# XinkeAE/Active-ORB-SLAM2

Hardware: AMD Instinct MI355X
Metric: frames/sec (extract+match+localBA) TUM 640x480 (higher is better)
Workload: dtype u8 (extract, match) + f64 (PoseOptimization, LocalBA)

## Files before the change

active-orb-slam2_amd/csrc/lba.hip:

```cpp
#include <dlfcn.h>

#include <chrono>
#include <cstdio>
#include <cstdlib>
#include <memory>
#include <numeric>
#include <atomic>
#include <condition_variable>
#include <functional>
#include <mutex>
#include <thread>

#include "lba_math.h"
#include "ldlt_reg.h"
#include "wave_ops.h"

namespace aos2 {

struct Cam {
    double fx, fy, cx, cy, bf;
    float bf_f;
    double delta_mono, delta_stereo;
};

struct LmState {
    double lambda, ni, currentChi, iniChi;
    double final_chi2, final_lambda;
    int32_t phase;
    int32_t run;
    int32_t lin;
    int32_t initp;
    int32_t xmark;
    int32_t it, qmax, nBad;
    int32_t iters_max[2], iters_done[2], trials[2];
    int32_t polls;
    int32_t stop_poll;
    int32_t stop_at_poll;
    int32_t n_active;
    int32_t solver_failed;
    int32_t blocks_done;
    int32_t ntr;
    int32_t err_at;
    int32_t pad_;
    double tr_rho[48], tr_temp[48], tr_cur[48], tr_lambda[48];
};

enum LdltForm : int { kLdltDev = 0, kLdltReg = 2 };

struct LbaWin {
    int n_poses, n_points, n_edges, np, nl, n_items;
    int iters1, iters2;
    const float *in_Tcw, *in_xyz, *in_obs, *in_w;
    double *pose, *point;
    double *bk;
    int est_n;
    const int32_t *e_pose, *e_point;
    const uint8_t *e_stereo;
    uint8_t *e_robust, *e_level1;
    double *err;
    Cam cam;
    const int32_t *pl_pos;
    const int32_t *hpose, *hpoint;
    const int32_t *pt_off, *pt_k;
    const int32_t *ps_off, *ps_k;
    const int32_t *pl_off, *pl_ph;
    const int32_t *it_ka, *it_kb, *it_l, *blk_off;
    const int32_t *sr_o0, *sr_info, *sr_ij;
    int n_srows;
    double *lrec;
    double *lomr;
    double *Rl;
    double *Hpp, *Hll, *b, *x, *Hs, *bs;
    double *tmp;
    double *scal;
    double *part;
    int n_part;
    double *ldlt;
    int npad;
    LdltForm ldlt_form;
    int hs_ld;
    LmState *st;
    const int32_t *abort_word;
    float *out_Tcw, *out_xyz;
    double *out_chi2;
    uint8_t *out_outlier;
};

static_assert(sizeof(LbaWin) == 520 && offsetof(LbaWin, st) == 472, "LbaWin's layout is fixed");

struct SchurTask {
    int32_t w;
    int32_t code;
};

__device__ inline bool lm_poll(LmState *st, const int32_t *abort_word, int seen = -1)
{
    st->polls++;
    if (st->stop_poll > 0) return true;
    const int a = seen >= 0 ? seen : abort_word ? __hip_atomic_load(abort_word, __ATOMIC_RELAXED, __HIP_MEMORY_SCOPE_SYSTEM) : 0;
    if (a || (st->stop_at_poll > 0 && st->polls >= st->stop_at_poll)) {
        st->stop_poll = st->polls;
        return true;
    }
    return false;
}

__device__ inline void lm_first_done(LmState *st, const int32_t *abort_word, int seen = -1)
{
    st->phase = 1;
    st->xmark = 0;
    if (lm_poll(st, abort_word, seen)) {
        st->phase = 3;
        return;
    }
    st->xmark = 1;
    st->n_active = 0;
}

template <int N>
__device__ __forceinline__ void workgroup_sum2(double v0, double v1, double *out0, double *out1)
{
    __shared__ double sh[2][N];
    sh[0][threadIdx.x] = v0;
    sh[1][threadIdx.x] = v1;
    __syncthreads();
#pragma unroll
    for (int s = N / 2; s > 0; s >>= 1) {
        if ((int)threadIdx.x < s) {
            sh[0][threadIdx.x] = sh[0][threadIdx.x] + sh[0][threadIdx.x + s];
            sh[1][threadIdx.x] = sh[1][threadIdx.x] + sh[1][threadIdx.x + s];
        }
        __syncthreads();
    }
    if (threadIdx.x == 0) {
        out0[blockIdx.x] = sh[0][0];
        out1[blockIdx.x] = sh[1][0];
    }
}

__global__ __launch_bounds__(256) void k_prepare(const LbaWin *__restrict__ wins, int stop_at_poll)
{
    const LbaWin &W = wins[blockIdx.y];
    const int i = blockIdx.x * 256 + threadIdx.x;
    if (i < W.n_poses) pose_from_Tcw(W.in_Tcw + 16 * (size_t)i, W.pose + 7 * (size_t)i);
    if (i < W.n_points)
        for (int d = 0; d < 3; ++d) W.point[3 * (size_t)i + d] = (double)W.in_xyz[3 * (size_t)i + d];
    if (i < W.n_edges) {
        for (int d = 0; d < 3; ++d) W.err[3 * (size_t)i + d] = 0.0;
        W.e_robust[i] = 1;
        W.e_level1[i] = 0;
    }
    if (blockIdx.x == 0 && W.hs_ld == W.npad) {
        const int n = 6 * W.np, npad = W.npad;
        for (int q = threadIdx.x; q < (npad - n) * npad; q += 256) {
            const int r = n + q / npad, c = q % npad;
            W.Hs[(size_t)r * npad + c] = r == c ? 1.0 : 0.0;
        }
        for (int q = threadIdx.x; q < n * (npad - n); q += 256) {
            const int r = q / (npad - n), c = n + q % (npad - n);
            W.Hs[(size_t)r * npad + c] = 0.0;
        }
    }
    if (blockIdx.x == 0) {
        LmState *st = W.st;
        static_assert(sizeof(LmState) % 8 == 0, "LmState is cleared as 64-bit words");
        for (int k = threadIdx.x; k < (int)(sizeof(LmState) / 8); k += 256) reinterpret_cast<long long *>(st)[k] = 0;
        __syncthreads();
        if (threadIdx.x == 0) {
            st->iters_max[0] = W.iters1;
            st->iters_max[1] = W.iters2;
            st->polls = 1;
            st->stop_at_poll = stop_at_poll;
            st->n_active = W.n_edges;
            st->phase = 0;
            st->it = 0;
            if (st->iters_max[0] <= 0 || lm_poll(st, W.abort_word)) {
                st->iters_done[0] = 0;
                lm_first_done(st, W.abort_word);
            } else
                st->initp = 1;
        }
    }
}
// ... 347 lines not shown
            const int a = e0 + kLmSlots * rd + j;
            double c = 0;
            if (a < e1) {
                const int e = W.pt_k[a];
                if (!W.e_level1[e]) {
                    double p[3], er[3];
                    se3_map(W.pose + 7 * (size_t)W.e_pose[e], Xv, p);
                    const int stereo = W.e_stereo[e];
                    const double ob[3] = {(double)W.in_obs[3 * (size_t)e], (double)W.in_obs[3 * (size_t)e + 1], (double)W.in_obs[3 * (size_t)e + 2]};
                    edge_error(W.cam, p, ob, stereo, er);
                    c = edge_chi2(er, (double)W.in_w[e], stereo ? 3 : 2);
                    if (W.e_robust[e]) {
                        double rho[2];
                        robustify(c, stereo ? W.cam.delta_stereo : W.cam.delta_mono, rho);
                        c = rho[0];
                    }
                }
            }
            s_v[ll][j][0] = c;
            __syncthreads();
            if (leader) {
                const int m = min(kLmSlots, e1 - (e0 + kLmSlots * rd));
                for (int jj = 0; jj < m; ++jj) chi += s_v[ll][jj][0];
            }
        }
    }
    if (has && leader) {
        store_dev(W.part + l, chi);
        store_dev(W.part + W.nl + l, sc);
    }
    if (solve) points_tail<256>(W);
}

__global__ __launch_bounds__(128) void k_points_walk(const LbaWin *__restrict__ wins, const SchurTask *__restrict__ tasks, int solve)
{
    const SchurTask tk = tasks[blockIdx.x];
    const LbaWin &W = wins[tk.w];
    if (!(solve ? W.st->run : W.st->initp)) return;
    const int l = tk.code * blockDim.x + threadIdx.x;
    const int n6 = 6 * W.np;
    if (l < W.nl) {
        double sc = 0, chi = 0;
        double *X = W.point + 3 * (size_t)W.hpoint[l];
        double Xv[3] = {X[0], X[1], X[2]};
        if (solve) {
            const double lambda = W.st->lambda;
            double cl[3] = {W.b[n6 + 3 * l], W.b[n6 + 3 * l + 1], W.b[n6 + 3 * l + 2]};
            const int a0 = W.pl_off[l], a1 = W.pl_off[l + 1];
            for (int a = a0; a < a1; a += kWalkChunk) {
                int ka[kWalkChunk], i1[kWalkChunk];
#pragma unroll
                for (int u = 0; u < kWalkChunk; ++u) ka[u] = min(a + u, a1 - 1);
#pragma unroll
                for (int u = 0; u < kWalkChunk; ++u) i1[u] = W.pl_ph[ka[u]];
                dbl4_t rec[kWalkChunk];
                double xp[kWalkChunk][6], Rr[kWalkChunk][9];
#pragma unroll
                for (int u = 0; u < kWalkChunk; ++u) rec[u] = lrec_load(W, ka[u]);
#pragma unroll
                for (int u = 0; u < kWalkChunk; ++u) {
#pragma unroll
                    for (int r = 0; r < 6; ++r) xp[u][r] = -W.x[6 * i1[u] + r];
#pragma unroll
                    for (int i = 0; i < 9; ++i) Rr[u][i] = W.Rl[9 * (size_t)i1[u] + i];
                }
#pragma unroll
                for (int u = 0; u < kWalkChunk; ++u) {
                    if (a + u >= a1) break;
                    double v[3];
                    lrec_backsub(W.cam, rec[u], Rr[u], xp[u], v);
                    for (int c = 0; c < 3; ++c) cl[c] += v[c];
                }
            }
            double Dm[9], Dinv[9];
            for (int i = 0; i < 9; ++i) Dm[i] = W.Hll[9 * (size_t)l + i];
            Dm[0] += lambda; Dm[4] += lambda; Dm[8] += lambda;
            mat3_inverse(Dm, Dinv);
            double *Xb = W.bk + 7 * (size_t)W.n_poses + 3 * (size_t)W.hpoint[l];
            for (int r = 0; r < 3; ++r) {
                const double xl = Dinv[r * 3] * cl[0] + Dinv[r * 3 + 1] * cl[1] + Dinv[r * 3 + 2] * cl[2];
                W.x[n6 + 3 * l + r] = xl;
                store_dev(Xb + r, Xv[r]);
                Xv[r] += xl;
                store_dev(X + r, Xv[r]);
                sc += xl * (lambda * xl + W.b[n6 + 3 * l + r]);
            }
        }
        const int e0 = W.pt_off[l], e1 = W.pt_off[l + 1];
        for (int a = e0; a < e1; a += kWalkChunkE) {
            int e[kWalkChunkE], ep[kWalkChunkE];
            uint8_t lv1[kWalkChunkE], ste[kWalkChunkE], rob[kWalkChunkE];
            double T[kWalkChunkE][7], ob[kWalkChunkE][3], ew[kWalkChunkE];
#pragma unroll
            for (int u = 0; u < kWalkChunkE; ++u) e[u] = W.pt_k[min(a + u, e1 - 1)];
#pragma unroll
            for (int u = 0; u < kWalkChunkE; ++u) {
                ep[u] = W.e_pose[e[u]];
                lv1[u] = W.e_level1[e[u]];
                ste[u] = W.e_stereo[e[u]];
                rob[u] = W.e_robust[e[u]];
                ew[u] = (double)W.in_w[e[u]];
#pragma unroll
                for (int i = 0; i < 3; ++i) ob[u][i] = (double)W.in_obs[3 * (size_t)e[u] + i];
            }
#pragma unroll
            for (int u = 0; u < kWalkChunkE; ++u)
#pragma unroll
                for (int i = 0; i < 7; ++i) T[u][i] = W.pose[7 * (size_t)ep[u] + i];
#pragma unroll
            for (int u = 0; u < kWalkChunkE; ++u) {
                if (a + u >= e1) break;
                if (lv1[u]) continue;
                double p[3], er[3];
                se3_map(T[u], Xv, p);
                const int stereo = ste[u];
                edge_error(W.cam, p, ob[u], stereo, er);
                double c = edge_chi2(er, ew[u], stereo ? 3 : 2);
                if (rob[u]) {
                    double rho[2];
                    robustify(c, stereo ? W.cam.delta_stereo : W.cam.delta_mono, rho);
                    c = rho[0];
                }
                chi += c;
            }
        }
        store_dev(W.part + l, chi);
        store_dev(W.part + W.nl + l, sc);
    }
    if (solve) points_tail<128>(W);
}

__device__ __forceinline__ void edge_weights_of(const Cam &cam, const double er[3], double w, int robust, int stereo, double omr[3], double &wo)
{
    omr[0] = -(w * er[0]);
    omr[1] = -(w * er[1]);
    omr[2] = stereo ? -(w * er[2]) : 0.0;
    wo = w;
    if (robust) {
        double rho[2];
        robustify(edge_chi2(er, w, stereo ? 3 : 2), stereo ? cam.delta_stereo : cam.delta_mono, rho);
        wo = rho[1] * w;
        omr[0] *= rho[1];
        omr[1] *= rho[1];
        if (stereo) omr[2] *= rho[1];
    }
}
__device__ __forceinline__ void edge_weights(const LbaWin &W, int k, const double p[3], int stereo, double omr[3], double &wo)
{
    const double ob[3] = {(double)W.in_obs[3 * (size_t)k], (double)W.in_obs[3 * (size_t)k + 1], (double)W.in_obs[3 * (size_t)k + 2]};
    double er[3];
    edge_error(W.cam, p, ob, stereo, er);
    edge_weights_of(W.cam, er, (double)W.in_w[k], W.e_robust[k], stereo, omr, wo);
}

__device__ __forceinline__ void lin_points_body(const LbaWin &W, int blk)
{
    __shared__ double s_c[kLmBlock][kLmSlots][12 + 1];
    const int tid = threadIdx.x, ll = tid / kLmSlots, j = tid % kLmSlots;
    const int l = blk * kLmBlock + ll;
    const bool has = l < W.nl, leader = j == 0;
    double Xv[3] = {0, 0, 0};
// ... 17 lines not shown
            jac_point(W.cam, R, p, stereo, Ja);
            double omr[3], wo;
            edge_weights(W, k, p, stereo, omr, wo);
#pragma unroll
            for (int r = 0; r < 3; ++r) {
                cb[r] = Ja[r] * omr[0] + Ja[3 + r] * omr[1] + Ja[6 + r] * omr[2];
#pragma unroll
                for (int c = 0; c < 3; ++c) cH[r * 3 + c] = Ja[r] * wo * Ja[c] + Ja[3 + r] * wo * Ja[3 + c] + Ja[6 + r] * wo * Ja[6 + c];
            }
            const int pp = W.pl_pos[k];
            if (pp >= 0) lrec_store(W, pp, p, wo, stereo, omr);
        }
#pragma unroll
        for (int i = 0; i < 9; ++i) s_c[ll][j][i] = cH[i];
#pragma unroll
        for (int i = 0; i < 3; ++i) s_c[ll][j][9 + i] = cb[i];
        __syncthreads();
        if (leader) {
            const int m = min(kLmSlots, a1 - (a0 + kLmSlots * rd));
            for (int jj = 0; jj < m; ++jj) {
#pragma unroll
                for (int i = 0; i < 9; ++i) H[i] += s_c[ll][jj][i];
#pragma unroll
                for (int i = 0; i < 3; ++i) bl[i] += s_c[ll][jj][9 + i];
            }
        }
    }
    if (has && leader) {
        for (int i = 0; i < 9; ++i) W.Hll[9 * (size_t)l + i] = H[i];
        for (int i = 0; i < 3; ++i) W.b[6 * (size_t)W.np + 3 * (size_t)l + i] = bl[i];
    }
}

__device__ __forceinline__ void lin_points_walk(const LbaWin &W, int l)
{
    if (l >= W.nl) return;
    const double *X = W.point + 3 * (size_t)W.hpoint[l];
    const double Xv[3] = {X[0], X[1], X[2]};
    double H[9] = {0, 0, 0, 0, 0, 0, 0, 0, 0}, bl[3] = {0, 0, 0};
    const int e0 = W.pt_off[l], e1 = W.pt_off[l + 1];
    for (int a = e0; a < e1; a += kWalkChunkLin) {
        int kk[kWalkChunkLin], ep[kWalkChunkLin], ph[kWalkChunkLin];
        uint8_t lv1[kWalkChunkLin], ste[kWalkChunkLin], rob[kWalkChunkLin];
        double T[kWalkChunkLin][7], er[kWalkChunkLin][3], ew[kWalkChunkLin];
#pragma unroll
        for (int u = 0; u < kWalkChunkLin; ++u) kk[u] = W.pt_k[min(a + u, e1 - 1)];
#pragma unroll
        for (int u = 0; u < kWalkChunkLin; ++u) {
            ep[u] = W.e_pose[kk[u]];
            ph[u] = W.pl_pos[kk[u]];
            lv1[u] = W.e_level1[kk[u]];
            ste[u] = W.e_stereo[kk[u]];
            rob[u] = W.e_robust[kk[u]];
            ew[u] = (double)W.in_w[kk[u]];
#pragma unroll
            for (int i = 0; i < 3; ++i) er[u][i] = (double)W.in_obs[3 * (size_t)kk[u] + i];
        }
#pragma unroll
        for (int u = 0; u < kWalkChunkLin; ++u)
#pragma unroll
            for (int i = 0; i < 7; ++i) T[u][i] = W.pose[7 * (size_t)ep[u] + i];
#pragma unroll
        for (int u = 0; u < kWalkChunkLin; ++u) {
            if (a + u >= e1) break;
            if (lv1[u]) continue;
            const int stereo = ste[u];
            double p[3], R[9];
            se3_map(T[u], Xv, p);
            rot_from_quat(T[u], R);
            double Ja[9];
            jac_point(W.cam, R, p, stereo, Ja);
            double omr[3], wo;
            double res[3];
            edge_error(W.cam, p, er[u], stereo, res);
            edge_weights_of(W.cam, res, ew[u], rob[u], stereo, omr, wo);
#pragma unroll
            for (int r = 0; r < 3; ++r) {
                bl[r] += Ja[r] * omr[0] + Ja[3 + r] * omr[1] + Ja[6 + r] * omr[2];
#pragma unroll
                for (int c = 0; c < 3; ++c) H[r * 3 + c] += Ja[r] * wo * Ja[c] + Ja[3 + r] * wo * Ja[3 + c] + Ja[6 + r] * wo * Ja[6 + c];
            }
            if (ph[u] >= 0) lrec_store(W, ph[u], p, wo, stereo, omr);
        }
    }
    for (int i = 0; i < 9; ++i) W.Hll[9 * (size_t)l + i] = H[i];
    for (int i = 0; i < 3; ++i) W.b[6 * (size_t)W.np + 3 * (size_t)l + i] = bl[i];
}

template <int K, int NT = 256>
__device__ __forceinline__ double workgroup_sum_k256(double (&acc)[K], double *red , int n_items)
{
    const int row = threadIdx.x >> 4, wave = threadIdx.x >> 6;
    const int rows_used = min(NT / 16, (n_items + 15) >> 4);
    if (wave * 64 < n_items) {
        row_sums_scatter_f64<K>(acc);
        row_scatter_store<K>(acc, red + row * (K + 1));
    }
    __syncthreads();
    double sum = 0;
    if ((int)threadIdx.x < K)
        for (int r = 0; r < rows_used; ++r) sum += red[r * (K + 1) + threadIdx.x];
    return sum;
}

__device__ __forceinline__ void lin_poses_body(const LbaWin &W, int ph, int init)
{
    __shared__ double red[16 * 43];
    if (ph >= W.np) return;
    double T[7];
    {
        const double *Tp = W.pose + 7 * (size_t)W.hpose[ph];
#pragma unroll
        for (int i = 0; i < 7; ++i) T[i] = Tp[i];
    }
    if (threadIdx.x == 0) {
        double R[9];
        rot_from_quat(T, R);
// ... 6 lines not shown
    for (int i = 0; i < 42; ++i) acc[i] = 0;
    for (int a = W.ps_off[ph] + threadIdx.x; a < W.ps_off[ph + 1]; a += 256) {
        const int k = W.ps_k[a];
        if (W.e_level1[k]) continue;
        const int stereo = W.e_stereo[k];
        double p[3], Jb[18], omr[3], wo;
        se3_map(T, W.point + 3 * (size_t)W.e_point[k], p);
        jac_pose(W.cam, p, stereo, Jb);
        edge_weights(W, k, p, stereo, omr, wo);
#pragma unroll
        for (int r = 0; r < 6; ++r) {
            acc[36 + r] += Jb[r] * omr[0] + Jb[6 + r] * omr[1] + Jb[12 + r] * omr[2];
#pragma unroll
            for (int c = 0; c < 6; ++c) acc[r * 6 + c] += Jb[r] * wo * Jb[c] + Jb[6 + r] * wo * Jb[6 + c] + Jb[12 + r] * wo * Jb[12 + c];
        }
    }
    const double sum = workgroup_sum_k256<42>(acc, red, W.ps_off[ph + 1] - W.ps_off[ph]);
    if (threadIdx.x < 36)
        W.Hpp[36 * (size_t)ph + threadIdx.x] = sum;
    else if (threadIdx.x < 42)
        W.b[6 * (size_t)ph + (threadIdx.x - 36)] = sum;
}

template <bool kWalk>
__global__ __launch_bounds__(256) __attribute__((amdgpu_waves_per_eu(3, 3))) void k_lin(const LbaWin *__restrict__ wins, const SchurTask *__restrict__ tasks, int init)
{
    const SchurTask tk = tasks[blockIdx.x];
    const LbaWin &W = wins[tk.w];
    if (!(init ? W.st->initp : W.st->lin)) return;
    const int blk = tk.code & 0x0fffffff;
    const bool keyframe = (tk.code >> 28) != 0;
    if (keyframe)
        lin_poses_body(W, blk, init);
    else if (kWalk)
        lin_points_walk(W, blk * 256 + threadIdx.x);
    else
        lin_points_body(W, blk);
}

__global__ __launch_bounds__(1024) void k_lm_init(const LbaWin *__restrict__ wins)
{
    __shared__ double sh[1024];
    const LbaWin &W = wins[blockIdx.x];
    LmState *st = W.st;
    if (!st->initp) return;
    const int n6 = 6 * W.np, n = n6 + 3 * W.nl;
    double acc = 0;
    for (int i = threadIdx.x; i < n; i += 1024) {
        double v;
        if (i < n6)
            v = W.Hpp[36 * (size_t)(i / 6) + (i % 6) * 7];
        else {
            const int j = i - n6;
            v = W.Hll[9 * (size_t)(j / 3) + (j % 3) * 4];
        }
        acc = fmax(acc, fabs(v));
    }
    sh[threadIdx.x] = acc;
    __syncthreads();
    for (int s = 512; s > 0; s >>= 1) {
        if ((int)threadIdx.x < s) sh[threadIdx.x] = fmax(sh[threadIdx.x], sh[threadIdx.x + s]);
        __syncthreads();
    }
    for (int i = threadIdx.x; i < W.est_n; i += 1024) W.bk[i] = W.pose[i];
    double chi, unused;
    canonical_sums(W, false, chi, unused);
    if (threadIdx.x == 0) {
        st->currentChi = st->iniChi = chi;
        st->lambda = 1e-5 * sh[0];
// ... 510 lines not shown
        for (int i = 0; i < 6; ++i) {
            upd[i] = xs[6 * tid + i];
            Wn.tmp[6 * tid + i] = upd[i] * (lambda * upd[i] + Wn.b[6 * tid + i]);
        }
        double *Tp = Wn.pose + 7 * (size_t)Wn.hpose[tid], *Tbk = Wn.bk + 7 * (size_t)Wn.hpose[tid];
        for (int i = 0; i < 7; ++i) Tbk[i] = Tp[i];
        se3_oplus_fast(upd, Tp);
    }
}

__device__ __forceinline__ void edge_last_error(const LbaWin &W, int e, int at, const double p_cur[3], int stereo, bool keep, double er[3])
{
    double *dst = W.err + 3 * (size_t)e;
    if (at == 0) {
        er[0] = dst[0]; er[1] = dst[1]; er[2] = dst[2];
        return;
    }
    double p[3] = {p_cur[0], p_cur[1], p_cur[2]};
    if (at == 2) se3_map(W.bk + 7 * (size_t)W.e_pose[e], W.bk + 7 * (size_t)W.n_poses + 3 * (size_t)W.e_point[e], p);
    const double ob[3] = {(double)W.in_obs[3 * (size_t)e], (double)W.in_obs[3 * (size_t)e + 1], (double)W.in_obs[3 * (size_t)e + 2]};
    edge_error(W.cam, p, ob, stereo, er);
    if (keep) {
        dst[0] = er[0]; dst[1] = er[1]; dst[2] = er[2];
    }
}

__global__ __launch_bounds__(256) void k_transition(const LbaWin *__restrict__ wins)
{
    __shared__ int s_last;
    const LbaWin &W = wins[blockIdx.y];
    LmState *st = W.st;
    if (!st->xmark) return;
    const int err_at = st->err_at;
    const int e = blockIdx.x * blockDim.x + threadIdx.x;
    int keep = 0;
    if (e < W.n_edges) {
        const int stereo = W.e_stereo[e];
        double p[3], er[3];
        se3_map(W.pose + 7 * (size_t)W.e_pose[e], W.point + 3 * (size_t)W.e_point[e], p);
        edge_last_error(W, e, err_at, p, stereo, true, er);
        const double c = edge_chi2(er, (double)W.in_w[e], stereo ? 3 : 2);
        const bool bad = c > (stereo ? 7.815 : 5.991) || !(p[2] > 0.0);
        if (bad) {
            W.e_level1[e] = 1;
            const int pp = W.pl_pos[e];
            if (pp >= 0) lrec_mask(W, pp);
        }
        W.e_robust[e] = 0;
        keep = bad ? 0 : 1;
    }
    const unsigned long long m = __ballot(keep);
    if ((threadIdx.x & 63) == 0 && m) atomicAdd(&st->n_active, __popcll(m));
    asm volatile("s_waitcnt vmcnt(0)" ::: "memory");
    __syncthreads();
    if (threadIdx.x == 0) s_last = __hip_atomic_fetch_add(&st->blocks_done, 1, __ATOMIC_RELAXED, __HIP_MEMORY_SCOPE_AGENT) == (int)gridDim.x - 1;
    __syncthreads();
    if (!s_last || threadIdx.x != 0) return;
    st->blocks_done = 0;
    st->xmark = 0;
    st->it = 0;
    st->err_at = 0;
    const int n_active = __hip_atomic_load(&st->n_active, __ATOMIC_RELAXED, __HIP_MEMORY_SCOPE_AGENT);
    if (n_active == 0 || st->iters_max[1] <= 0 || lm_poll(st, W.abort_word)) {
        st->phase = 3;
        st->iters_done[1] = 0;
    } else {
        st->phase = 2;
        st->initp = 1;
    }
}

__global__ __launch_bounds__(256) void k_final(const LbaWin *__restrict__ wins)
{
    const LbaWin &W = wins[blockIdx.y];
    const int i = blockIdx.x * blockDim.x + threadIdx.x;
    if (i < W.n_edges) {
        const int stereo = W.e_stereo[i];
        double p[3], er[3];
        se3_map(W.pose + 7 * (size_t)W.e_pose[i], W.point + 3 * (size_t)W.e_point[i], p);
        edge_last_error(W, i, W.e_level1[i] ? 0 : W.st->err_at, p, stereo, false, er);
        const double c = edge_chi2(er, (double)W.in_w[i], stereo ? 3 : 2);
// ... 254 lines not shown
    const int np = S.np;
    for (int i = 0; i < np; ++i) S.units.push_back((kSchurDiag << 28) | i);
    std::vector<int32_t> pack_first;
    int in_unit = 0;
    for (int i1 = 0, blk = 0; i1 < np; ++i1)
        for (int i2 = i1; i2 < np; ++i2, ++blk) {
            if (i2 == i1) continue;
            const int o0 = S.blk_off[blk], n = S.blk_off[blk + 1] - o0;
            if (n > 256) {
                S.units.push_back((kSchurBig << 28) | blk);
                continue;
            }
            const int nrows = std::max(1, (n + 15) / 16);
            if (in_unit + nrows > 16) {
                for (; in_unit < 16; ++in_unit) {
                    S.sr_o0.push_back(0); S.sr_info.push_back(0); S.sr_ij.push_back(0);
                }
                in_unit = 0;
            }
            if (in_unit == 0) pack_first.push_back((int32_t)S.sr_o0.size());
            for (int r = 0; r < nrows; ++r) {
                S.sr_o0.push_back(o0 + 16 * r);
                S.sr_info.push_back(std::max(0, std::min(16, n - 16 * r)) | (r << 8) | (nrows << 16));
                S.sr_ij.push_back(i1 | (i2 << 16));
            }
            in_unit = (in_unit + nrows) % 16;
        }
    for (int32_t f : pack_first) S.units.push_back((kSchurPack << 28) | f);
}

struct WinLayout {
    size_t in_Tcw, in_xyz, in_obs, in_w, e_pose, e_point, e_stereo, pl_pos, hpose, hpoint, pt_off, pt_k, ps_off, ps_k,
        pl_off, pl_k, it_ka, it_kb, it_l, blk_off, sr_o0, sr_info, sr_ij;
    size_t est, bk, robust, level1, err, lrec, lomr, Rl, Hpp, Hll, b, x, Hs, bs, tmp, scal, part, ldlt;
    size_t out_Tcw, out_xyz, out_outlier, out_chi2, st;
    int n_part, npad;
    LdltForm ldlt_form;
    size_t n_items;
};

struct RoctxRange {
    typedef int (*push_t)(const char *);
    typedef int (*pop_t)();
    static void resolve(push_t &push, pop_t &pop)
    {
        static push_t s_push = nullptr;
        static pop_t s_pop = nullptr;
        static bool tried = false;
        if (!tried) {
            tried = true;
            const char *v = getenv("AOS2_ROCTX");
            if (v && atoi(v) != 0) {
                void *h = dlopen("librocprofiler-sdk-roctx.so", RTLD_NOW | RTLD_GLOBAL);
                if (!h) h = dlopen("libroctx64.so", RTLD_NOW | RTLD_GLOBAL);
                if (h) {
                    s_push = (push_t)dlsym(h, "roctxRangePushA");
                    s_pop = (pop_t)dlsym(h, "roctxRangePop");
                }
            }
        }
        push = s_push;
        pop = s_pop;
    }
    pop_t pop_ = nullptr;
    explicit RoctxRange(const char *name)
    {
        push_t push;
// ... 76 lines not shown
    list(l.blk_off, S.blk_off, 4);
    list(l.sr_o0, S.sr_o0, 4); list(l.sr_info, S.sr_info, 4); list(l.sr_ij, S.sr_ij, 4);
}

static void layout_staged(const aos2_lba_problem_t &p, const Pass &S, Bump &B, WinLayout &l)
{
    for_each_staged(p, S, l, [&](size_t &off, const void *, size_t bytes, size_t tail) { off = B.take(bytes + tail); });
    l.n_items = S.it_ka.size();
}

static void stage_window(uint8_t *dst, const WinLayout &l, const aos2_lba_problem_t &p, const Pass &S)
{
    for_each_staged(p, S, l, [&](size_t off, const void *src, size_t bytes, size_t) {
        if (bytes) memcpy(dst + off, src, bytes);
    });
}

static void layout_scratch(const aos2_lba_problem_t &p, const Pass &S, const LmLayout &lay, Bump &B, WinLayout &l)
{
    const size_t NP = p.n_poses, NL = p.n_points, E = p.n_edges;
    const size_t n6 = 6 * (size_t)S.np, dim = n6 + 3 * (size_t)S.nl;
    l.est = B.take(8 * (7 * NP + 3 * NL)); l.bk = B.take(8 * (7 * NP + 3 * NL));
    l.robust = B.take(E); l.level1 = B.take(E);
    l.err = B.take(24 * E);
    l.lrec = B.take(32 * (S.pl_k.size() + 1)); l.lomr = B.take(24 * (S.pl_k.size() + 1)); l.Rl = B.take(72 * (size_t)S.np + 8);
    l.Hpp = B.take(288 * (size_t)S.np + 8); l.Hll = B.take(72 * (size_t)S.nl + 8);
    l.b = B.take(8 * dim + 8); l.x = B.take(8 * dim + 8);
    l.npad = (int)((n6 + 15) & ~(size_t)15);
    l.ldlt_form = l.npad <= 16 * kLrMaxNb ? kLdltReg : kLdltDev;
    l.Hs = B.take(8 * (size_t)l.npad * l.npad + 8); l.bs = B.take(8 * n6 + 8);
    l.tmp = B.take(8 * n6 + 8);
    l.n_part = lay.points_blocks(S);
    l.scal = B.take(64); l.part = B.take(16 * (size_t)std::max(S.nl, 1) + 8);
    l.ldlt = B.take(8);
}

static void layout_results(const aos2_lba_problem_t &p, bool want_chi2, Bump &B, WinLayout &l)
{
    const size_t NP = p.n_poses, NL = p.n_points, E = p.n_edges;
    l.st = B.take(sizeof(LmState), 64);
    l.out_Tcw = B.take(64 * NP, 64); l.out_xyz = B.take(12 * NL, 64); l.out_outlier = B.take(E, 64);
    l.out_chi2 = want_chi2 ? B.take(8 * E, 64) : 0;
}

static void describe_window(LbaWin &W, uint8_t *base, const aos2_lba_problem_t &p, const Pass &S, const WinLayout &l, const int32_t *abort_word, bool want_chi2)
{
    memset(&W, 0, sizeof(W));
    W.n_poses = p.n_poses; W.n_points = p.n_points; W.n_edges = p.n_edges;
    W.np = S.np; W.nl = S.nl; W.n_items = (int)l.n_items;
    W.iters1 = p.iters_first; W.iters2 = p.iters_second;
    W.in_Tcw = (const float *)(base + l.in_Tcw); W.in_xyz = (const float *)(base + l.in_xyz);
    W.in_obs = (const float *)(base + l.in_obs); W.in_w = (const float *)(base + l.in_w);
    W.pose = (double *)(base + l.est); W.point = W.pose + 7 * (size_t)p.n_poses;
    W.bk = (double *)(base + l.bk);
    W.est_n = 7 * p.n_poses + 3 * p.n_points;
    W.e_pose = (const int32_t *)(base + l.e_pose); W.e_point = (const int32_t *)(base + l.e_point);
    W.e_stereo = base + l.e_stereo; W.e_robust = base + l.robust; W.e_level1 = base + l.level1;
    W.err = (double *)(base + l.err);
    W.cam.fx = (double)p.fx; W.cam.fy = (double)p.fy; W.cam.cx = (double)p.cx; W.cam.cy = (double)p.cy;
    W.cam.bf = (double)p.bf; W.cam.bf_f = p.bf;
    W.cam.delta_mono = (double)(float)std::sqrt(5.991);
    W.cam.delta_stereo = (double)(float)std::sqrt(7.815);
    W.pl_pos = (const int32_t *)(base + l.pl_pos);
    W.hpose = (const int32_t *)(base + l.hpose); W.hpoint = (const int32_t *)(base + l.hpoint);
    W.pt_off = (const int32_t *)(base + l.pt_off); W.pt_k = (const int32_t *)(base + l.pt_k);
    W.ps_off = (const int32_t *)(base + l.ps_off); W.ps_k = (const int32_t *)(base + l.ps_k);
    W.pl_off = (const int32_t *)(base + l.pl_off); W.pl_ph = (const int32_t *)(base + l.pl_k);
    W.it_ka = (const int32_t *)(base + l.it_ka); W.it_kb = (const int32_t *)(base + l.it_kb);
    W.it_l = (const int32_t *)(base + l.it_l); W.blk_off = (const int32_t *)(base + l.blk_off);
    W.sr_o0 = (const int32_t *)(base + l.sr_o0); W.sr_info = (const int32_t *)(base + l.sr_info); W.sr_ij = (const int32_t *)(base + l.sr_ij);
    W.n_srows = (int)S.sr_o0.size();
    W.lrec = (double *)(base + l.lrec); W.lomr = (double *)(base + l.lomr); W.Rl = (double *)(base + l.Rl); W.Hpp = (double *)(base + l.Hpp);
    W.Hll = (double *)(base + l.Hll); W.b = (double *)(base + l.b); W.x = (double *)(base + l.x);
    W.Hs = (double *)(base + l.Hs); W.bs = (double *)(base + l.bs);
    W.tmp = (double *)(base + l.tmp); W.scal = (double *)(base + l.scal); W.part = (double *)(base + l.part);
    W.n_part = l.n_part;
    W.ldlt = (double *)(base + l.ldlt); W.npad = l.npad; W.ldlt_form = l.ldlt_form;
    W.hs_ld = l.npad;
    W.st = (LmState *)(base + l.st);
    W.abort_word = abort_word;
    W.out_Tcw = (float *)(base + l.out_Tcw); W.out_xyz = (float *)(base + l.out_xyz);
    W.out_outlier = base + l.out_outlier;
    W.out_chi2 = want_chi2 ? (double *)(base + l.out_chi2) : nullptr;
}


struct GroupDims {
    bool any_glob = false, any_reg = false;
    int mx_E = 0, mx_pts = 0, mx_npad_glob = 0, mx_npad_reg = 0;
    void add(const aos2_lba_problem_t &p, const Pass &S, const WinLayout &l)
    {
        if (S.np > 0) {
            if (l.ldlt_form == kLdltReg) {
                any_reg = true;
                mx_npad_reg = std::max(mx_npad_reg, l.npad);
            } else {
                any_glob = true;
                mx_npad_glob = std::max(mx_npad_glob, l.npad);
            }
        }
        mx_E = std::max(mx_E, p.n_edges);
        mx_pts = std::max(mx_pts, std::max(p.n_points, p.n_poses));
    }
};

struct TaskLists {
    std::vector<SchurTask> schur, pts, lin;
    size_t size() const { return schur.size() + pts.size() + lin.size(); }
};

static void build_tasks(const std::vector<Pass> &passes, const std::vector<int> &ids, bool by_position, const LmLayout &lay, TaskLists &T, bool one_queue = false)
{
    auto wmap = [&](int k) { return by_position ? k : ids[k]; };
    std::vector<SchurTask> &tasks = T.schur;
    const int nwg = (int)ids.size();
    std::vector<int> order(nwg);
    std::iota(order.begin(), order.end(), 0);
    auto weight = [&](int k) { return passes[ids[k]].units.size(); };
    std::stable_sort(order.begin(), order.end(), [&](int a, int b) { return weight(a) > weight(b); });
    const int NX = nwg >= 8 && !one_queue ? 8 : 1;
    std::vector<std::vector<int>> xw(NX);
    std::vector<size_t> load(NX, 0);
    for (int k : order) {
        const int x = (int)(std::min_element(load.begin(), load.end()) - load.begin());
        xw[x].push_back(k);
        load[x] += weight(k);
    }
    std::vector<std::vector<SchurTask>> qx(NX);
    for (int x = 0; x < NX; ++x)
        for (size_t k = 0; k < xw[x].size(); k += 2) {
            const int a = xw[x][k], b = k + 1 < xw[x].size() ? xw[x][k + 1] : -1;
            const std::vector<int32_t> &ua = passes[ids[a]].units;
            static const std::vector<int32_t> none;
            const std::vector<int32_t> &ub = b >= 0 ? passes[ids[b]].units : none;
            for (size_t u = 0; u < std::max(ua.size(), ub.size()); ++u) {
// ... 45 lines not shown

struct StreamSet {
    hipStream_t q, q2;
    hipEvent_t fork, join;
};
static StreamSet group_streams(const aos2_lba *s, int g)
{
    return g == 0 ? StreamSet{s->stream, s->stream2, s->ev_fork, s->ev_join} : StreamSet{s->stream_b, s->stream2_b, s->ev_fork_b, s->ev_join_b};
}

struct Prog : StreamSet {
    const LbaWin *wins, *blk;
    int nw;
    const SchurTask *schur, *pts, *lin;
    size_t n_schur, n_pts, n_lin;
    GroupDims D;
};
static Prog make_prog(const LbaWin *wins, const LbaWin *blk, int nw, const TaskLists &T, const DevTasks &d, const GroupDims &D, const StreamSet &Q)
{
    return Prog{Q, wins, blk, nw, d.schur, d.pts, d.lin, T.schur.size(), T.pts.size(), T.lin.size(), D};
}

struct LaunchCtx {
    aos2_lba *s;
    bool walk;
    bool stagger_pending;
};

static unsigned blocks(size_t n, int t) { return (unsigned)((n + t - 1) / t); }

static void enqueue_points(const LaunchCtx &C, const Prog &P, int solve)
{
    if (C.walk)
        hipLaunchKernelGGL(k_points_walk, dim3((unsigned)P.n_pts), dim3(128), 0, P.q, P.wins, P.pts, solve);
    else
        hipLaunchKernelGGL(k_points, dim3((unsigned)P.n_pts), dim3(256), 0, P.q, P.wins, P.pts, solve);
}
static void enqueue_lin(const LaunchCtx &C, const Prog &P, int init)
{
    if (!P.n_lin) return;
    if (C.walk)
        hipLaunchKernelGGL(k_lin<true>, dim3((unsigned)P.n_lin), dim3(256), 0, P.q, P.wins, P.lin, init);
    else
        hipLaunchKernelGGL(k_lin<false>, dim3((unsigned)P.n_lin), dim3(256), 0, P.q, P.wins, P.lin, init);
}
static void enqueue_init(const LaunchCtx &C, const Prog &P)
{
    enqueue_points(C, P, 0);
    enqueue_lin(C, P, 1);
    hipLaunchKernelGGL(k_lm_init, dim3(P.nw), dim3(1024), 0, P.q, P.blk);
}
static void enqueue_schur(const Prog &P)
{
    if (P.n_schur) hipLaunchKernelGGL(k_schur, dim3((unsigned)P.n_schur), dim3(kSchurThreads), 0, P.q, P.wins, P.schur);
}
static void enqueue_trial(LaunchCtx &C, const Prog &P, bool first_group)
{
    const GroupDims &D = P.D;
    enqueue_schur(P);
    if (first_group && C.stagger_pending) {
        (void)hipEventRecord(C.s->ev_stag, C.s->stream);
        (void)hipStreamWaitEvent(C.s->stream_b, C.s->ev_stag, 0);
        C.stagger_pending = false;
    }
    const bool both = D.any_glob && D.any_reg;
    if (both) {
        (void)hipEventRecord(P.fork, P.q);
        (void)hipStreamWaitEvent(P.q2, P.fork, 0);
    }
    enqueue_ldlt(P.blk, P.nw, D.any_reg ? D.mx_npad_reg : 0, D.any_glob ? D.mx_npad_glob : 0, both ? P.q2 : P.q, P.q);
    if (both) {
        (void)hipEventRecord(P.join, P.q2);
        (void)hipStreamWaitEvent(P.q, P.join, 0);
    }
    enqueue_points(C, P, 1);
// ... 707 lines not shown
```

Baseline: 77070.

## Pack per-edge data into 32-byte records and stage pose/x/Rl in LDS

```diff
diff --git a/active-orb-slam2_amd/csrc/lba.hip b/active-orb-slam2_amd/csrc/lba.hip
--- a/active-orb-slam2_amd/csrc/lba.hip
+++ b/active-orb-slam2_amd/csrc/lba.hip
@@ -46,6 +46,16 @@
 };
 
 enum LdltForm : int { kLdltDev = 0, kLdltReg = 2 };
+
+struct EdgeRec {
+    float obs[3], w;
+    int32_t pose;
+    int32_t pl_pos;
+    uint32_t flags;
+    uint32_t pad_;
+};
+static_assert(sizeof(EdgeRec) == 32, "an edge record is two 16-byte loads");
+constexpr uint32_t kEdgeStereo = 1, kEdgeRobust = 2, kEdgeLevel1 = 4;
 
 struct LbaWin {
     int n_poses, n_points, n_edges, np, nl, n_items;
@@ -75,7 +85,7 @@
     double *scal;
     double *part;
     int n_part;
-    double *ldlt;
+    EdgeRec *erec;
     int npad;
     LdltForm ldlt_form;
     int hs_ld;
@@ -93,6 +103,21 @@
     int32_t code;
 };
 
+typedef float flt4_t __attribute__((ext_vector_type(4)));
+typedef int int4_t __attribute__((ext_vector_type(4)));
+__device__ __forceinline__ void erec_load(const LbaWin &W, int a, flt4_t &lo, int4_t &hi)
+{
+    const EdgeRec *r = W.erec + a;
+    lo = *reinterpret_cast<const flt4_t *>(r);
+    hi = *(reinterpret_cast<const int4_t *>(r) + 1);
+}
+__device__ __forceinline__ void erec_store(const LbaWin &W, int a, flt4_t lo, int4_t hi)
+{
+    EdgeRec *r = W.erec + a;
+    *reinterpret_cast<flt4_t *>(r) = lo;
+    *(reinterpret_cast<int4_t *>(r) + 1) = hi;
+}
+
 __device__ inline bool lm_poll(LmState *st, const int32_t *abort_word, int seen = -1)
 {
     st->polls++;
@@ -149,6 +174,10 @@
         for (int d = 0; d < 3; ++d) W.err[3 * (size_t)i + d] = 0.0;
         W.e_robust[i] = 1;
         W.e_level1[i] = 0;
+        const int k = W.pt_k[i];
+        const flt4_t lo = {W.in_obs[3 * (size_t)k], W.in_obs[3 * (size_t)k + 1], W.in_obs[3 * (size_t)k + 2], W.in_w[k]};
+        const int4_t hi = {W.e_pose[k], W.pl_pos[k], (int)((W.e_stereo[k] ? kEdgeStereo : 0) | kEdgeRobust), 0};
+        erec_store(W, i, lo, hi);
     }
     if (blockIdx.x == 0 && W.hs_ld == W.npad) {
         const int n = 6 * W.np, npad = W.npad;
@@ -562,101 +591,126 @@
     if (solve) points_tail<256>(W);
 }
 
+constexpr int kWalkLdsBytes = 16 * 1024;
+extern __shared__ double walk_sm[];
+__host__ __device__ constexpr int walk_lds_bytes(int n_poses, int np) { return 8 * (7 * n_poses + 15 * np); }
+__device__ __forceinline__ void walk_stage(const LbaWin &W, double *sm, bool with_x)
+{
+    const int n7 = 7 * W.n_poses, n6 = 6 * W.np, n9 = 9 * W.np;
+    for (int i = threadIdx.x; i < n7; i += blockDim.x) sm[i] = W.pose[i];
+    if (with_x) {
+        for (int i = threadIdx.x; i < n6; i += blockDim.x) sm[n7 + i] = W.x[i];
+        for (int i = threadIdx.x; i < n9; i += blockDim.x) sm[n7 + n6 + i] = W.Rl[i];
+    }
+    __syncthreads();
+}
+
+template <bool kLds>
+__device__ __forceinline__ void points_walk_body(const LbaWin &W, int l, int solve, int hp, int a0, int a1, int e0, int e1)
+{
+    const int n6 = 6 * W.np;
+    const double *s_pose = walk_sm, *s_x = walk_sm + 7 * W.n_poses, *s_Rl = s_x + n6;
+    double sc = 0, chi = 0;
+    double *X = W.point + 3 * (size_t)hp;
+    double Xv[3] = {X[0], X[1], X[2]};
+    if (solve) {
+        const double lambda = W.st->lambda;
+        double cl[3] = {W.b[n6 + 3 * l], W.b[n6 + 3 * l + 1], W.b[n6 + 3 * l + 2]};
+        for (int a = a0; a < a1; a += kWalkChunk) {
+            int ka[kWalkChunk], i1[kWalkChunk];
+#pragma unroll
+            for (int u = 0; u < kWalkChunk; ++u) ka[u] = min(a + u, a1 - 1);
+#pragma unroll
+            for (int u = 0; u < kWalkChunk; ++u) i1[u] = W.pl_ph[ka[u]];
+            dbl4_t rec[kWalkChunk];
+            double xp[kWalkChunk][6], Rr[kWalkChunk][9];
+#pragma unroll
+            for (int u = 0; u < kWalkChunk; ++u) rec[u] = lrec_load(W, ka[u]);
+#pragma unroll
+            for (int u = 0; u < kWalkChunk; ++u) {
+#pragma unroll
+                for (int r = 0; r < 6; ++r) xp[u][r] = -(kLds ? s_x[6 * i1[u] + r] : W.x[6 * i1[u] + r]);
+#pragma unroll
+                for (int i = 0; i < 9; ++i) Rr[u][i] = kLds ? s_Rl[9 * i1[u] + i] : W.Rl[9 * (size_t)i1[u] + i];
+            }
+#pragma unroll
+            for (int u = 0; u < kWalkChunk; ++u) {
+                if (a + u >= a1) break;
+                double v[3];
+                lrec_backsub(W.cam, rec[u], Rr[u], xp[u], v);
+                for (int c = 0; c < 3; ++c) cl[c] += v[c];
+            }
+        }
+        double Dm[9], Dinv[9];
+        for (int i = 0; i < 9; ++i) Dm[i] = W.Hll[9 * (size_t)l + i];
+        Dm[0] += lambda; Dm[4] += lambda; Dm[8] += lambda;
+        mat3_inverse(Dm, Dinv);
+        double *Xb = W.bk + 7 * (size_t)W.n_poses + 3 * (size_t)hp;
+        for (int r = 0; r < 3; ++r) {
+            const double xl = Dinv[r * 3] * cl[0] + Dinv[r * 3 + 1] * cl[1] + Dinv[r * 3 + 2] * cl[2];
+            W.x[n6 + 3 * l + r] = xl;
+            store_dev(Xb + r, Xv[r]);
+            Xv[r] += xl;
+            store_dev(X + r, Xv[r]);
+            sc += xl * (lambda * xl + W.b[n6 + 3 * l + r]);
+        }
+    }
+    for (int a = e0; a < e1; a += kWalkChunkE) {
+        flt4_t lo[kWalkChunkE];
+        int4_t hi[kWalkChunkE];
+        double T[kWalkChunkE][7];
+#pragma unroll
+        for (int u = 0; u < kWalkChunkE; ++u) erec_load(W, min(a + u, e1 - 1), lo[u], hi[u]);
+#pragma unroll
+        for (int u = 0; u < kWalkChunkE; ++u)
+#pragma unroll
+            for (int i = 0; i < 7; ++i) T[u][i] = kLds ? s_pose[7 * hi[u].x + i] : W.pose[7 * (size_t)hi[u].x + i];
+#pragma unroll
+        for (int u = 0; u < kWalkChunkE; ++u) {
+            if (a + u >= e1) break;
+            const uint32_t fl = (uint32_t)hi[u].z;
+            if (fl & kEdgeLevel1) continue;
+            double p[3], er[3];
+            se3_map(T[u], Xv, p);
+            const int stereo = fl & kEdgeStereo;
+            const double ob[3] = {(double)lo[u].x, (double)lo[u].y, (double)lo[u].z};
+            edge_error(W.cam, p, ob, stereo, er);
+            double c = edge_chi2(er, (double)lo[u].w, stereo ? 3 : 2);
+            if (fl & kEdgeRobust) {
+                double rho[2];
+                robustify(c, stereo ? W.cam.delta_stereo : W.cam.delta_mono, rho);
+                c = rho[0];
+            }
+            chi += c;
+        }
+    }
+    store_dev(W.part + l, chi);
+    store_dev(W.part + W.nl + l, sc);
+}
+
 __global__ __launch_bounds__(128) void k_points_walk(const LbaWin *__restrict__ wins, const SchurTask *__restrict__ tasks, int solve)
 {
     const SchurTask tk = tasks[blockIdx.x];
     const LbaWin &W = wins[tk.w];
     if (!(solve ? W.st->run : W.st->initp)) return;
     const int l = tk.code * blockDim.x + threadIdx.x;
-    const int n6 = 6 * W.np;
-    if (l < W.nl) {
-        double sc = 0, chi = 0;
-        double *X = W.point + 3 * (size_t)W.hpoint[l];
-        double Xv[3] = {X[0], X[1], X[2]};
+    const bool has = l < W.nl;
+    int hp = 0, a0 = 0, a1 = 0, e0 = 0, e1 = 0;
+    if (has) {
+        hp = W.hpoint[l];
+        e0 = W.pt_off[l];
+        e1 = W.pt_off[l + 1];
         if (solve) {
-            const double lambda = W.st->lambda;
-            double cl[3] = {W.b[n6 + 3 * l], W.b[n6 + 3 * l + 1], W.b[n6 + 3 * l + 2]};
-            const int a0 = W.pl_off[l], a1 = W.pl_off[l + 1];
-            for (int a = a0; a < a1; a += kWalkChunk) {
-                int ka[kWalkChunk], i1[kWalkChunk];
-#pragma unroll
-                for (int u = 0; u < kWalkChunk; ++u) ka[u] = min(a + u, a1 - 1);
-#pragma unroll
-                for (int u = 0; u < kWalkChunk; ++u) i1[u] = W.pl_ph[ka[u]];
-                dbl4_t rec[kWalkChunk];
-                double xp[kWalkChunk][6], Rr[kWalkChunk][9];
-#pragma unroll
-                for (int u = 0; u < kWalkChunk; ++u) rec[u] = lrec_load(W, ka[u]);
-#pragma unroll
-                for (int u = 0; u < kWalkChunk; ++u) {
-#pragma unroll
-                    for (int r = 0; r < 6; ++r) xp[u][r] = -W.x[6 * i1[u] + r];
-#pragma unroll
-                    for (int i = 0; i < 9; ++i) Rr[u][i] = W.Rl[9 * (size_t)i1[u] + i];
-                }
-#pragma unroll
-                for (int u = 0; u < kWalkChunk; ++u) {
-                    if (a + u >= a1) break;
-                    double v[3];
-                    lrec_backsub(W.cam, rec[u], Rr[u], xp[u], v);
-                    for (int c = 0; c < 3; ++c) cl[c] += v[c];
-                }
-            }
-            double Dm[9], Dinv[9];
-            for (int i = 0; i < 9; ++i) Dm[i] = W.Hll[9 * (size_t)l + i];
-            Dm[0] += lambda; Dm[4] += lambda; Dm[8] += lambda;
-            mat3_inverse(Dm, Dinv);
-            double *Xb = W.bk + 7 * (size_t)W.n_poses + 3 * (size_t)W.hpoint[l];
-            for (int r = 0; r < 3; ++r) {
-                const double xl = Dinv[r * 3] * cl[0] + Dinv[r * 3 + 1] * cl[1] + Dinv[r * 3 + 2] * cl[2];
-                W.x[n6 + 3 * l + r] = xl;
-                store_dev(Xb + r, Xv[r]);
-                Xv[r] += xl;
-                store_dev(X + r, Xv[r]);
-                sc += xl * (lambda * xl + W.b[n6 + 3 * l + r]);
-            }
-        }
-        const int e0 = W.pt_off[l], e1 = W.pt_off[l + 1];
-        for (int a = e0; a < e1; a += kWalkChunkE) {
-            int e[kWalkChunkE], ep[kWalkChunkE];
-            uint8_t lv1[kWalkChunkE], ste[kWalkChunkE], rob[kWalkChunkE];
-            double T[kWalkChunkE][7], ob[kWalkChunkE][3], ew[kWalkChunkE];
-#pragma unroll
-            for (int u = 0; u < kWalkChunkE; ++u) e[u] = W.pt_k[min(a + u, e1 - 1)];
-#pragma unroll
-            for (int u = 0; u < kWalkChunkE; ++u) {
-                ep[u] = W.e_pose[e[u]];
-                lv1[u] = W.e_level1[e[u]];
-                ste[u] = W.e_stereo[e[u]];
-                rob[u] = W.e_robust[e[u]];
-                ew[u] = (double)W.in_w[e[u]];
-#pragma unroll
-                for (int i = 0; i < 3; ++i) ob[u][i] = (double)W.in_obs[3 * (size_t)e[u] + i];
-            }
-#pragma unroll
-            for (int u = 0; u < kWalkChunkE; ++u)
-#pragma unroll
-                for (int i = 0; i < 7; ++i) T[u][i] = W.pose[7 * (size_t)ep[u] + i];
-#pragma unroll
-            for (int u = 0; u < kWalkChunkE; ++u) {
-                if (a + u >= e1) break;
-                if (lv1[u]) continue;
-                double p[3], er[3];
-                se3_map(T[u], Xv, p);
-                const int stereo = ste[u];
-                edge_error(W.cam, p, ob[u], stereo, er);
-                double c = edge_chi2(er, ew[u], stereo ? 3 : 2);
-                if (rob[u]) {
-                    double rho[2];
-                    robustify(c, stereo ? W.cam.delta_stereo : W.cam.delta_mono, rho);
-                    c = rho[0];
-                }
-                chi += c;
-            }
-        }
-        store_dev(W.part + l, chi);
-        store_dev(W.part + W.nl + l, sc);
-    }
+            a0 = W.pl_off[l];
+            a1 = W.pl_off[l + 1];
+        }
+    }
+    const bool lds = walk_lds_bytes(W.n_poses, W.np) <= kWalkLdsBytes;
+    if (lds) {
+        walk_stage(W, walk_sm, solve != 0);
+        if (has) points_walk_body<true>(W, l, solve, hp, a0, a1, e0, e1);
+    } else if (has)
+        points_walk_body<false>(W, l, solve, hp, a0, a1, e0, e1);
     if (solve) points_tail<128>(W);
 }
 
@@ -740,39 +794,31 @@
     }
 }
 
+template <bool kLds>
 __device__ __forceinline__ void lin_points_walk(const LbaWin &W, int l)
 {
-    if (l >= W.nl) return;
+    const double *s_pose = walk_sm;
+    const int e0 = W.pt_off[l], e1 = W.pt_off[l + 1];
     const double *X = W.point + 3 * (size_t)W.hpoint[l];
     const double Xv[3] = {X[0], X[1], X[2]};
     double H[9] = {0, 0, 0, 0, 0, 0, 0, 0, 0}, bl[3] = {0, 0, 0};
-    const int e0 = W.pt_off[l], e1 = W.pt_off[l + 1];
     for (int a = e0; a < e1; a += kWalkChunkLin) {
-        int kk[kWalkChunkLin], ep[kWalkChunkLin], ph[kWalkChunkLin];
-        uint8_t lv1[kWalkChunkLin], ste[kWalkChunkLin], rob[kWalkChunkLin];
-        double T[kWalkChunkLin][7], er[kWalkChunkLin][3], ew[kWalkChunkLin];
-#pragma unroll
-        for (int u = 0; u < kWalkChunkLin; ++u) kk[u] = W.pt_k[min(a + u, e1 - 1)];
-#pragma unroll
-        for (int u = 0; u < kWalkChunkLin; ++u) {
-            ep[u] = W.e_pose[kk[u]];
-            ph[u] = W.pl_pos[kk[u]];
-            lv1[u] = W.e_level1[kk[u]];
-            ste[u] = W.e_stereo[kk[u]];
-            rob[u] = W.e_robust[kk[u]];
-            ew[u] = (double)W.in_w[kk[u]];
-#pragma unroll
-            for (int i = 0; i < 3; ++i) er[u][i] = (double)W.in_obs[3 * (size_t)kk[u] + i];
-        }
+        flt4_t lo[kWalkChunkLin];
+        int4_t hi[kWalkChunkLin];
+        double T[kWalkChunkLin][7];
+#pragma unroll
+        for (int u = 0; u < kWalkChunkLin; ++u) erec_load(W, min(a + u, e1 - 1), lo[u], hi[u]);
 #pragma unroll
         for (int u = 0; u < kWalkChunkLin; ++u)
 #pragma unroll
-            for (int i = 0; i < 7; ++i) T[u][i] = W.pose[7 * (size_t)ep[u] + i];
+            for (int i = 0; i < 7; ++i) T[u][i] = kLds ? s_pose[7 * hi[u].x + i] : W.pose[7 * (size_t)hi[u].x + i];
 #pragma unroll
         for (int u = 0; u < kWalkChunkLin; ++u) {
             if (a + u >= e1) break;
-            if (lv1[u]) continue;
-            const int stereo = ste[u];
+            const uint32_t fl = (uint32_t)hi[u].z;
+            if (fl & kEdgeLevel1) continue;
+            const int stereo = fl & kEdgeStereo;
+            const double ob[3] = {(double)lo[u].x, (double)lo[u].y, (double)lo[u].z};
             double p[3], R[9];
             se3_map(T[u], Xv, p);
             rot_from_quat(T[u], R);
@@ -780,17 +826,18 @@
             jac_point(W.cam, R, p, stereo, Ja);
             double omr[3], wo;
             double res[3];
-            edge_error(W.cam, p, er[u], stereo, res);
-            edge_weights_of(W.cam, res, ew[u], rob[u], stereo, omr, wo);
+            edge_error(W.cam, p, ob, stereo, res);
+            edge_weights_of(W.cam, res, (double)lo[u].w, (fl & kEdgeRobust) != 0, stereo, omr, wo);
 #pragma unroll
             for (int r = 0; r < 3; ++r) {
                 bl[r] += Ja[r] * omr[0] + Ja[3 + r] * omr[1] + Ja[6 + r] * omr[2];
 #pragma unroll
                 for (int c = 0; c < 3; ++c) H[r * 3 + c] += Ja[r] * wo * Ja[c] + Ja[3 + r] * wo * Ja[3 + c] + Ja[6 + r] * wo * Ja[6 + c];
             }
-            if (ph[u] >= 0) lrec_store(W, ph[u], p, wo, stereo, omr);
-        }
-    }
+            if (hi[u].y >= 0) lrec_store(W, hi[u].y, p, wo, stereo, omr);
+        }
+    }
+    asm volatile("" : "+v"(l));
     for (int i = 0; i < 9; ++i) W.Hll[9 * (size_t)l + i] = H[i];
     for (int i = 0; i < 3; ++i) W.b[6 * (size_t)W.np + 3 * (size_t)l + i] = bl[i];
 }
@@ -863,9 +910,15 @@
     const bool keyframe = (tk.code >> 28) != 0;
     if (keyframe)
         lin_poses_body(W, blk, init);
-    else if (kWalk)
-        lin_points_walk(W, blk * 256 + threadIdx.x);
-    else
+    else if (kWalk) {
+        const int l = blk * 256 + threadIdx.x;
+        const bool has = l < W.nl;
+        if (walk_lds_bytes(W.n_poses, W.np) <= kWalkLdsBytes) {
+            walk_stage(W, walk_sm, false);
+            if (has) lin_points_walk<true>(W, l);
+        } else if (has)
+            lin_points_walk<false>(W, l);
+    } else
         lin_points_body(W, blk);
 }
 
@@ -1442,9 +1495,10 @@
     LmState *st = W.st;
     if (!st->xmark) return;
     const int err_at = st->err_at;
-    const int e = blockIdx.x * blockDim.x + threadIdx.x;
+    const int a = blockIdx.x * blockDim.x + threadIdx.x;
     int keep = 0;
-    if (e < W.n_edges) {
+    if (a < W.n_edges) {
+        const int e = W.pt_k[a];
         const int stereo = W.e_stereo[e];
         double p[3], er[3];
         se3_map(W.pose + 7 * (size_t)W.e_pose[e], W.point + 3 * (size_t)W.e_point[e], p);
@@ -1457,6 +1511,7 @@
             if (pp >= 0) lrec_mask(W, pp);
         }
         W.e_robust[e] = 0;
+        W.erec[a].flags = (W.erec[a].flags & ~kEdgeRobust) | (bad ? kEdgeLevel1 : 0);
         keep = bad ? 0 : 1;
     }
     const unsigned long long m = __ballot(keep);
@@ -1777,7 +1832,7 @@
 struct WinLayout {
     size_t in_Tcw, in_xyz, in_obs, in_w, e_pose, e_point, e_stereo, pl_pos, hpose, hpoint, pt_off, pt_k, ps_off, ps_k,
         pl_off, pl_k, it_ka, it_kb, it_l, blk_off, sr_o0, sr_info, sr_ij;
-    size_t est, bk, robust, level1, err, lrec, lomr, Rl, Hpp, Hll, b, x, Hs, bs, tmp, scal, part, ldlt;
+    size_t est, bk, robust, level1, err, lrec, lomr, Rl, Hpp, Hll, b, x, Hs, bs, tmp, scal, part, erec;
     size_t out_Tcw, out_xyz, out_outlier, out_chi2, st;
     int n_part, npad;
     LdltForm ldlt_form;
@@ -1920,7 +1975,7 @@
     l.tmp = B.take(8 * n6 + 8);
     l.n_part = lay.points_blocks(S);
     l.scal = B.take(64); l.part = B.take(16 * (size_t)std::max(S.nl, 1) + 8);
-    l.ldlt = B.take(8);
+    l.erec = B.take(sizeof(EdgeRec) * (E + 1));
 }
 
 static void layout_results(const aos2_lba_problem_t &p, bool want_chi2, Bump &B, WinLayout &l)
@@ -1963,7 +2018,7 @@
     W.Hs = (double *)(base + l.Hs); W.bs = (double *)(base + l.bs);
     W.tmp = (double *)(base + l.tmp); W.scal = (double *)(base + l.scal); W.part = (double *)(base + l.part);
     W.n_part = l.n_part;
-    W.ldlt = (double *)(base + l.ldlt); W.npad = l.npad; W.ldlt_form = l.ldlt_form;
+    W.erec = (EdgeRec *)(base + l.erec); W.npad = l.npad; W.ldlt_form = l.ldlt_form;
     W.hs_ld = l.npad;
     W.st = (LmState *)(base + l.st);
     W.abort_word = abort_word;
@@ -1976,6 +2031,7 @@
 struct GroupDims {
     bool any_glob = false, any_reg = false;
     int mx_E = 0, mx_pts = 0, mx_npad_glob = 0, mx_npad_reg = 0;
+    int walk_lds = 0;
     void add(const aos2_lba_problem_t &p, const Pass &S, const WinLayout &l)
     {
         if (S.np > 0) {
@@ -1989,6 +2045,7 @@
         }
         mx_E = std::max(mx_E, p.n_edges);
         mx_pts = std::max(mx_pts, std::max(p.n_points, p.n_poses));
+        if (walk_lds_bytes(p.n_poses, S.np) <= kWalkLdsBytes) walk_lds = std::max(walk_lds, walk_lds_bytes(p.n_poses, S.np));
     }
 };
 
@@ -2100,7 +2157,7 @@
 static void enqueue_points(const LaunchCtx &C, const Prog &P, int solve)
 {
     if (C.walk)
-        hipLaunchKernelGGL(k_points_walk, dim3((unsigned)P.n_pts), dim3(128), 0, P.q, P.wins, P.pts, solve);
+        hipLaunchKernelGGL(k_points_walk, dim3((unsigned)P.n_pts), dim3(128), (size_t)P.D.walk_lds, P.q, P.wins, P.pts, solve);
     else
         hipLaunchKernelGGL(k_points, dim3((unsigned)P.n_pts), dim3(256), 0, P.q, P.wins, P.pts, solve);
 }
@@ -2108,7 +2165,7 @@
 {
     if (!P.n_lin) return;
     if (C.walk)
-        hipLaunchKernelGGL(k_lin<true>, dim3((unsigned)P.n_lin), dim3(256), 0, P.q, P.wins, P.lin, init);
+        hipLaunchKernelGGL(k_lin<true>, dim3((unsigned)P.n_lin), dim3(256), (size_t)P.D.walk_lds, P.q, P.wins, P.lin, init);
     else
         hipLaunchKernelGGL(k_lin<false>, dim3((unsigned)P.n_lin), dim3(256), 0, P.q, P.wins, P.lin, init);
 }
```

Measured after the change: 79270 (median of 6 runs). 1.03x the previous value.
